# NVlabs/CenterPose

Measured on NVIDIA H100. Metric: images/sec at 512x512 DLA-34 (dla_34 + DCNv2, 7 heads, decode + PnP), higher is better.
Workload: dtype tf32x3

## Files before the change

### centerpose_b200/csrc/common.cuh

```cuda
#pragma once
#include <cuda_runtime.h>
#include <stdint.h>
#include <stdio.h>
#include <string>

#include "../../include/centerpose_b200.h"

namespace cp {

void set_error(const std::string& msg);
int fail(int code, const std::string& msg);
extern thread_local long long g_launch_counter;

#define CP_CUDA_CHECK(expr)                                                              \
  do {                                                                                   \
    cudaError_t _e = (expr);                                                             \
    if (_e != cudaSuccess)                                                               \
      return ::cp::fail(CP_ERR_CUDA, std::string(#expr) + ": " + cudaGetErrorString(_e)); \
  } while (0)

#define CP_LAUNCH_CHECK(what)                                                            \
  do {                                                                                   \
    cudaError_t _e = cudaGetLastError();                                                 \
    if (_e != cudaSuccess)                                                               \
// ... 40 lines not shown
  const float* fuse_b[16];
  float* fuse_out[16];
  int fuse_cout[16];
  int ipm;
  long long wstride, tstride;
  unsigned nchw_per_model;
};
inline int model_ipm(const IgemmParams& p) { return p.ipm > 0 ? p.ipm : p.B; }

int launch_igemm_fp32(const IgemmParams& p, cudaStream_t stream);

int decode_pnp_models(const cp_decode_params* prm, int models, const cp_heads* heads, const double* meta, float* dets,
                      float* poses, int32_t* n_valid, void* workspace, size_t workspace_bytes, void* stream);

struct LaunchInfo {
  int BN = 0;
  int ksplit = 1;
  long long grid = 0;
};

bool conv3_c16_supported(const IgemmParams& p);
int launch_conv3_c16(const IgemmParams& p, cudaStream_t stream);
bool stem_supported(const IgemmParams& p);
int launch_stem_conv(const IgemmParams& p, cudaStream_t s);

struct ConvKernel {
  int family = CP_FAM_IGEMM_FP32;
  bool x3 = false;
  bool round_out = false;
  int BN = 0;
  int cslab = 0;
  size_t wbytes = 0;
};
struct ConvPolicy {
  bool small_on_cuda_cores;
  bool dcn_tma;
  bool round_out;
  bool cuda_core_fallback;
};
inline bool known_precision(int32_t precision) {
  return precision == CP_PREC_FP32 || precision == CP_PREC_TF32X3 || precision == CP_PREC_BF16 || precision == CP_PREC_TF32;
}
inline bool gather_x3(int32_t precision) { return precision == CP_PREC_TF32 || precision == CP_PREC_TF32X3; }
ConvKernel select_conv_kernel(const IgemmParams& p, int32_t precision, const ConvPolicy& pol);
struct alignas(64) TmaMaps {
  unsigned char map[4][128];
};
int conv_encode(const ConvKernel& k, const IgemmParams& p, int Bmax, TmaMaps* maps);
int conv_pack(const ConvKernel& k, const IgemmParams& p, int ld, void* tiles, cudaStream_t s);
int conv_launch(const ConvKernel& k, const IgemmParams& p, const TmaMaps* maps, cudaStream_t s, LaunchInfo* info = nullptr);
int run_conv(IgemmParams& p, int32_t precision, const ConvPolicy& pol, cudaStream_t s);

int splitk_factor(long long tiles, int slabs, int num_sms, size_t tile_floats, size_t ws_floats);

bool umma_supported(const IgemmParams& p, int prec);
int umma_tile_n(int CoutPad, int prec);
size_t umma_weight_bytes(int Kreal, int CoutPad, int prec);
int launch_pack_umma_weight(const float* src_k_by_ld, int ld, int Kreal, int Cout, int CoutPad, int prec, void* dst,
                            cudaStream_t s);
int launch_igemm_umma(const IgemmParams& p, int prec, cudaStream_t stream, LaunchInfo* info = nullptr);

int launch_maxpool2(const float* in, float* out, int B, int H, int W, int C, cudaStream_t s);
int launch_maxpool3s2(const float* in, const float* residual, float* out, int B, int H, int W, int C, cudaStream_t s);
int launch_pack_deconv_weight(const float* w_io44, const float* scale, float* out, int Cin, int Cout, int CoutPad, int Kpad,
                              cudaStream_t s);
int launch_upsample_add(const float* in, const float* wgt_kkc, const float* skip, float* out, int B,
                        int Hin, int Win, int C, int f, cudaStream_t s, int ipm = 0, long long wstride = 0);
int launch_pack_conv_weight(const float* w_oihw, const float* scale, float* out, int Cout, int Cin,
                            int kh, int kw, int CoutPad, int Kpad, int ld, int colOff, cudaStream_t s,
                            int CinPad = 0);
int launch_pack_bias(const float* conv_bias, const float* bn_w, const float* bn_b, const float* bn_mean,
                     const float* bn_var, float* scale_out, float* bias_out, int C, int CPad, float eps,
                     cudaStream_t s);
int launch_pack_up_weight(const float* w_c1kk, float* out_kkc, int C, int k, cudaStream_t s);
int launch_nchw_to_nhwc(const float* in, float* out, int B, int C, int H, int W, int outStride,
                        int chanOffset, cudaStream_t s);
int launch_nhwc_to_nchw(const float* in, float* out, int B, int C, int H, int W, int inStride, cudaStream_t s);
constexpr int kGnBlocks = 64, kGnMaxGroups = 64;
inline size_t gn_workspace_doubles(int B) { return (size_t)B * kGnMaxGroups * 2 * (1 + kGnBlocks); }
int launch_group_norm_relu(float* x, const float* gamma, const float* beta, int B, int HW, int C,
                           int stride, int chanOffset, int groups, float eps, double* ws, cudaStream_t s, int ipm = 0,
                           long long wstride = 0);
int launch_gru_gates(const float* xi, const float* hh, const float* hprev, float* hout, int B_HW, int C,
                     int first_step, cudaStream_t s);

constexpr int kX3GroupBlocks = 1;

bool tma_conv_supported(const IgemmParams& p, int x3);
size_t tma_weight_bytes(int Cin, int taps, int CoutPad, int x3);
int tma_tile_n(int CoutPad, int x3);
int tma_cslab(const IgemmParams& p, int x3);
int launch_pack_tma_weight(const float* src_k_by_ld, int ld, int Cin, int taps, int Cout, int CoutPad, int x3, int cslab,
                           int bn, void* dst, cudaStream_t s);
int tma_encode_nhwc_box(const float* base, int C, int W, int H, int B, int strideFloats, int boxC, int boxW, int boxH,
                        int swizzle64, void* map_out );
int tma_conv_encode(const IgemmParams& p, int Bmax, int cslab, void* maps_out );
int launch_conv_tma(const IgemmParams& p, const void* maps, const ConvKernel& k, cudaStream_t stream, LaunchInfo* info);

bool dcn_tma_supported(const IgemmParams& p, int x3);
int dcn_tma_tile_n(int CoutPad, int x3);
int dcn_tma_encode(const IgemmParams& p, int Bmax, void* map_out );
int launch_dcn_tma(const IgemmParams& p, const void* map, const ConvKernel& k, cudaStream_t stream, LaunchInfo* info);

inline int round_up(int x, int m) { return (x + m - 1) / m * m; }

extern thread_local int g_pdl;
// ... 45 lines not shown
```

### centerpose_b200/csrc/conv_select.cu

```cuda
#include <stdlib.h>

#include "common.cuh"

namespace cp {

ConvKernel select_conv_kernel(const IgemmParams& p, int32_t precision, const ConvPolicy& pol) {
  const bool small = p.mode == IGEMM_NCHW_SCALAR || p.Cin < 32;
  if (precision != CP_PREC_FP32 && !(pol.small_on_cuda_cores && small)) {
    const bool tma = precision == CP_PREC_TF32 || precision == CP_PREC_TF32X3;
    const bool x3 = precision == CP_PREC_TF32X3;
    if (tma && pol.dcn_tma && dcn_tma_supported(p, x3))
      return {CP_FAM_DCN_TMA, x3, pol.round_out && !x3, dcn_tma_tile_n(p.CoutPad, x3), 16,
              tma_weight_bytes(p.Cin, 9, p.CoutPad, x3)};
    if (tma && tma_conv_supported(p, x3))
      return {CP_FAM_CONV_TMA, x3, pol.round_out && !x3, tma_tile_n(p.CoutPad, x3), tma_cslab(p, x3),
              tma_weight_bytes(p.Cin, p.kh * p.kw, p.CoutPad, x3)};
    const bool gx3 = gather_x3(precision);
    const int phases = p.mode == IGEMM_DECONV ? 4 : 1;
    if (umma_supported(p, gx3))
      return {CP_FAM_IGEMM_UMMA, gx3, false, umma_tile_n(p.CoutPad, gx3), 0,
              phases * umma_weight_bytes(p.kh * p.kw * p.Cin, p.CoutPad, gx3)};
    if (!pol.cuda_core_fallback) return {CP_FAM_NONE};
  }
  return {stem_supported(p) ? CP_FAM_STEM : (conv3_c16_supported(p) ? CP_FAM_CONV3_C16 : CP_FAM_IGEMM_FP32)};
// ... 12 lines not shown
      return launch_pack_tma_weight(p.wgt, ld, p.Cin, p.kh * p.kw, p.Cout, p.CoutPad, k.x3, k.cslab, k.BN, tiles, s);
    case CP_FAM_IGEMM_UMMA: {
      const int phases = p.mode == IGEMM_DECONV ? 4 : 1;
      const size_t phase_bytes = k.wbytes / phases;
      for (int ph = 0; ph < phases; ++ph)
        if (int rc = launch_pack_umma_weight(p.wgt + (size_t)ph * p.Kpad * ld, ld, p.kh * p.kw * p.Cin, p.Cout, p.CoutPad,
                                             k.x3, (unsigned char*)tiles + ph * phase_bytes, s))
          return rc;
      return CP_OK;
    }
    default:
      return CP_OK;
  }
}

int conv_launch(const ConvKernel& k, const IgemmParams& p, const TmaMaps* maps, cudaStream_t s, LaunchInfo* info) {
  switch (k.family) {
    case CP_FAM_DCN_TMA: return launch_dcn_tma(p, maps->map, k, s, info);
    case CP_FAM_CONV_TMA: return launch_conv_tma(p, maps->map, k, s, info);
    case CP_FAM_IGEMM_UMMA: return launch_igemm_umma(p, k.x3, s, info);
    case CP_FAM_STEM: return launch_stem_conv(p, s);
    case CP_FAM_CONV3_C16: return launch_conv3_c16(p, s);
    case CP_FAM_IGEMM_FP32: return launch_igemm_fp32(p, s);
    default: return fail(CP_ERR_INVALID, "conv: no kernel selected");
  }
}

int run_conv(IgemmParams& p, int32_t precision, const ConvPolicy& pol, cudaStream_t s) {
  const ConvKernel k = select_conv_kernel(p, precision, pol);
  if (k.family == CP_FAM_NONE) return fail(CP_ERR_INVALID, "shape not supported by the wgmma kernel");
  if (!k.wbytes) return conv_launch(k, p, nullptr, s);
  void* tiles = nullptr;
  CP_CUDA_CHECK(cudaMallocAsync(&tiles, k.wbytes, s));
  TmaMaps maps;
  int rc = conv_encode(k, p, p.B, &maps);
  if (!rc) rc = conv_pack(k, p, p.CoutPad, tiles, s);
  if (!rc) {
    p.wgt_umma = tiles;
    rc = conv_launch(k, p, &maps, s);
  }
  cudaFreeAsync(tiles, s);
  return rc;
}

int splitk_factor(long long tiles, int slabs, int num_sms, size_t tile_floats, size_t ws_floats) {
  const char* off = getenv("CP_NO_SPLITK");
  if (!ws_floats || (off && atoi(off) != 0)) return 1;
  int S = 1;
  for (int cand = 2; cand <= slabs; ++cand)
    if (slabs % cand == 0 && tiles * cand <= num_sms && (size_t)tiles * cand * tile_floats <= ws_floats) S = cand;
  return S;
}

}
```

### centerpose_b200/csrc/conv_tma.cu

```cuda
#include <cuda.h>

#include "common.cuh"
#include "umma_common.cuh"

namespace cp {
namespace {

constexpr int TM_BM = 128;
constexpr int TM_THREADS = 384;
constexpr int TM_THREADS_X3 = 512;

struct TmaConvParams {
  CUtensorMap amap[4];
  int nsrc;
  int srcC[4];
  int B, H, W, Cin, Cout, CoutPad, BN;
  int k;
  int tile_m;
  int Wt, boxh;
  int tiles_per_image;
  long long total_tiles;
  long long m_tiles;
  uint32_t slab_bytes, slab_stride;
  int SA, SB;
  const float* bias;
  const float* residual;
  int resStride, relu, res_after_relu;
  float* out;
  int outStride, out_nchw;
  int round_tf32;
  int cslab;
  int x3;
  int group;
  const unsigned char* wtiles;
  int ksplit, sps;
  float* part;
  int fuse, tph;
  const float* fuse_w[16];
  const float* fuse_b[16];
  float* fuse_out[16];
  int fuse_cout[16];
  int ipm;
  long long wstride, tstride, tiles_per_model;
};

using namespace umma;

struct TmaCtl {
  unsigned long long a_full[4], a_empty[4], a_split[4];
  unsigned long long b_full[8], b_empty[8];
};
static_assert(sizeof(TmaCtl) <= 512, "control block");

struct TileGeo {
  int n_tile, img, g0, r_lo, model;
  long long pos0;
};
template <bool MULTI>
__device__ __forceinline__ TileGeo decode_tile(const TmaConvParams& p, long long ct, int n_tiles) {
  TileGeo g;
  g.n_tile = (int)(ct % n_tiles);
  const long long m_tile = ct / n_tiles;
  g.img = 0;
  g.g0 = 0;
  g.r_lo = 0;
  g.pos0 = 0;
  g.model = 0;
  if (p.k == 3) {
    g.img = (int)(m_tile / p.tiles_per_image);
    g.g0 = (int)(m_tile - (long long)g.img * p.tiles_per_image) * p.tile_m;
    const int t = g.g0 - 1;
    g.r_lo = (t >= 0) ? t / p.Wt : -((-t + p.Wt - 1) / p.Wt);
    if (MULTI) g.model = g.img / p.ipm;
  } else if (MULTI) {
    g.model = (int)(m_tile / p.tiles_per_model);
    g.pos0 = (long long)g.model * p.ipm * p.H * p.W + (m_tile - g.model * p.tiles_per_model) * p.tile_m;
  } else {
    g.pos0 = m_tile * p.tile_m;
  }
  return g;
}

template <bool MULTI>
__device__ __forceinline__ bool tile_position(const TmaConvParams& p, const TileGeo& g, int i, int* n, int* oy, int* ox, int* m) {
  bool valid;
  if (p.k == 3) {
// ... 137 lines not shown
              h.y = tf32_round(v[u].y); l.y = tf32_round(v[u].y - h.y);
              h.z = tf32_round(v[u].z); l.z = tf32_round(v[u].z - h.z);
              h.w = tf32_round(v[u].w); l.w = tf32_round(v[u].w - h.w);
              st_shared_v4f(hi + ((c0 + u * 128) << 4), h.x, h.y, h.z, h.w);
              st_shared_v4f(lo + ((c0 + u * 128) << 4), l.x, l.y, l.z, l.w);
            }
          }
        }
        fence_proxy_async_smem();
        mbar_arrive(smem_u32(&ctl->a_split[stage]));
        if (++stage == p.SA) {
          stage = 0;
          phase ^= 1u;
        }
      }
    }
  } else {
    if (X3) asm volatile("setmaxnreg.inc.sync.aligned.u32 208;");
    const int c = (warp - 4) >> 2, wt = tid & 127;
    float* dstage = reinterpret_cast<float*>(smem + (drain0 - smem_u32(smem))) + (size_t)c * (DRAIN_STAGE_BYTES / 4);
    const uint32_t bar_a = smem_u32(X3 ? &ctl->a_split[0] : &ctl->a_full[0]);
    const uint32_t bar_a_empty = smem_u32(&ctl->a_empty[0]);
    const uint32_t bar_b_full = smem_u32(&ctl->b_full[0]), bar_b_empty = smem_u32(&ctl->b_empty[0]);
    const uint32_t a_lo_u = p.slab_stride >> 4, b_lo_u = ((uint32_t)BN * rowb) >> 4;
    EpiParams ep;
    ep.bias = p.bias;
    ep.residual = p.residual;
    ep.resStride = p.resStride;
    ep.relu = p.relu;
    ep.res_after_relu = p.res_after_relu;
    ep.round_tf32 = p.round_tf32;
    ep.out = p.out;
    ep.outStride = p.outStride;
    ep.out_nchw = p.out_nchw;
    ep.Cout = p.Cout;
    ep.CoutPad = p.CoutPad;
    ep.H = p.H;
    ep.W = p.W;
    int sa = 0, sb = 0;
    uint32_t pa = 0, pb = 0;
    float acc[BN / 2];
    float sums[X3 ? BN / 2 : 1];
    float acc2[FUSE ? 16 : 1];
#pragma unroll
    for (int j = 0; j < BN / 2; ++j) acc[j] = 0.f;
#pragma unroll
    for (int j = 0; j < (FUSE ? 16 : 1); ++j) acc2[j] = 0.f;
    for (long long it = 0, tile = tile_at(0); tile < total_tiles; tile = tile_at(++it)) {
      const TileGeo g = decode_tile<MULTI>(p, tile / KS_SPLIT, n_tiles);
      const uint32_t row0 = (p.k == 3 ? (uint32_t)(g.g0 - 1 - g.r_lo * p.Wt) : 0u) + (uint32_t)c * 64u;
#pragma unroll
      for (int j = 0; j < (X3 ? BN / 2 : 1); ++j) sums[j] = 0.f;
      int kbi = 0, gk = 0;
      for (int s = 0; s < sps; ++s) {
        mbar_wait(bar_a + 8u * (uint32_t)sa, pa);
        const uint32_t a_slab = slabs0 + (uint32_t)sa * a_stage;
        for (int tap = 0; tap < taps; ++tap, ++kbi) {
          const int ky = tap / 3, kx = tap - ky * 3;
          const uint32_t arow = row0 + (p.k == 3 ? (uint32_t)(ky * p.Wt + kx) : 0u);
          mbar_wait(bar_b_full + 8u * (uint32_t)sb, pb);
          const uint64_t da = make_desc(a_slab + arow * rowb, p.cslab);
          const uint64_t db = make_desc(btiles0 + (uint32_t)sb * btile_bytes, p.cslab);
          const bool fresh = X3 ? gk == 0 : kbi == 0;
          if (p.cslab == 32)
            mma_kblock<BN, X3, false, 4>(acc, da, db, a_lo_u, b_lo_u, fresh);
          else
            mma_kblock<BN, X3, false, 2>(acc, da, db, a_lo_u, b_lo_u, fresh);
          if (wt == 0) {
            mbar_arrive(bar_b_empty + 8u * (uint32_t)sb);
            if (tap == taps - 1) mbar_arrive(bar_a_empty + 8u * (uint32_t)sa);
          }
          if (++sb == p.SB) {
            sb = 0;
            pb ^= 1u;
          }
          if (X3) {
            if (gk == p.group - 1 || kbi == KB - 1) {
#pragma unroll
              for (int j = 0; j < (X3 ? BN / 2 : 1); ++j) sums[j] += acc[X3 ? j : 0];
              gk = 0;
            } else {
              ++gk;
            }
          }
        }
        if (++sa == p.SA) {
          sa = 0;
          pa ^= 1u;
        }
      }
      const int r_me = wt >> 1;
      int n, oy, ox, m;
      const bool valid = tile_position<MULTI>(p, g, c * 64 + r_me, &n, &oy, &ox, &m);
      const int col_end = min(p.Cout, (g.n_tile + 1) * BN);
      const int head = FUSE ? g.n_tile / p.tph : 0, part = FUSE ? g.n_tile - head * p.tph : 0;
      const size_t wofs = MULTI ? (size_t)g.model * p.wstride : 0;
      if (MULTI) ep.bias = p.bias + wofs;
      if (FUSE && part == 0) {
#pragma unroll
        for (int j = 0; j < (FUSE ? 16 : 1); ++j) acc2[j] = 0.f;
      }
      auto fn = [&](int r, int cb, float (&v)[16]) {
        if (cb >= BN) return;
        if (!FUSE && KS_SPLIT > 1) {
          const long long mn = tile / KS_SPLIT;
          const int ks = (int)(tile % KS_SPLIT);
          float4* mine = reinterpret_cast<float4*>(p.part) + (((size_t)mn * KS_SPLIT + ks) * (BN >> 2) + (cb >> 2)) * p.tile_m +
                         c * 64 + r;
#pragma unroll
          for (int q = 0; q < 4; ++q) __stcg(mine + (size_t)q * p.tile_m, make_float4(v[4 * q], v[4 * q + 1], v[4 * q + 2], v[4 * q + 3]));
        } else if (FUSE) {
          const float* b1 = p.bias + wofs + (size_t)g.n_tile * BN + cb;
          const float4* w2 = reinterpret_cast<const float4*>(p.fuse_w[head] + wofs) + ((size_t)part * BN + cb) * 4;
#pragma unroll
          for (int q = 0; q < 16; ++q) {
            const float h = fmaxf(v[q] + __ldg(b1 + q), 0.f);
#pragma unroll
            for (int u = 0; u < 4; ++u) {
              const float4 w = __ldg(w2 + q * 4 + u);
              acc2[FUSE ? 4 * u + 0 : 0] = fmaf(h, w.x, acc2[FUSE ? 4 * u + 0 : 0]);
              acc2[FUSE ? 4 * u + 1 : 0] = fmaf(h, w.y, acc2[FUSE ? 4 * u + 1 : 0]);
              acc2[FUSE ? 4 * u + 2 : 0] = fmaf(h, w.z, acc2[FUSE ? 4 * u + 2 : 0]);
              acc2[FUSE ? 4 * u + 3 : 0] = fmaf(h, w.w, acc2[FUSE ? 4 * u + 3 : 0]);
            }
          }
        } else {
          epilogue_row<16>(ep, v, valid, m, n, oy, ox, g.n_tile * BN + cb, col_end);
        }
      };
      if constexpr (X3)
        drain_rows<BN>(sums, dstage, wt, 1 + c, fn);
      else
        drain_rows<BN>(acc, dstage, wt, 1 + c, fn);
      if (FUSE && part == p.tph - 1) {
#pragma unroll
        for (int j = 0; j < (FUSE ? 16 : 1); ++j) acc2[j] += __shfl_xor_sync(0xffffffffu, acc2[j], 1);
        if ((wt & 1) == 0 && valid) {
          const int co = p.fuse_cout[head];
          float* o = p.fuse_out[head] + ((size_t)n * co * p.H + oy) * p.W + ox;
          const size_t plane = (size_t)p.H * p.W;
#pragma unroll
          for (int j = 0; j < 16; ++j)
            if (j < co) o[j * plane] = acc2[FUSE ? j : 0] + __ldg(p.fuse_b[head] + wofs + j);
// ... 203 lines not shown
  cudaLaunchConfig_t cfg = cfg0;
  cudaLaunchAttribute attr[1];
  attr[0].id = cudaLaunchAttributeProgrammaticStreamSerialization;
  attr[0].val.programmaticStreamSerializationAllowed = 1;
  cfg.attrs = attr;
  cfg.numAttrs = g_pdl ? 1 : 0;
  CP_CUDA_CHECK(cudaLaunchKernelEx(&cfg, kern, q));
  CP_LAUNCH_CHECK("conv_tma_kernel");
  return CP_OK;
}

int launch_conv_tma(const IgemmParams& p, const void* maps, const ConvKernel& k, cudaStream_t stream, LaunchInfo* info) {
  if (!p.wgt_umma) return fail(CP_ERR_INVALID, "conv_tma: weight tiles missing");
  if (p.B % model_ipm(p)) return fail(CP_ERR_INVALID, "conv_tma: batch is not a whole number of models");
  const bool x3 = k.x3;
  TmaConvParams q;
  memset(&q, 0, sizeof(q));
  memcpy(q.amap, maps, sizeof(CUtensorMap) * 4);
  q.nsrc = p.nsrc;
  for (int s = 0; s < 4; ++s) q.srcC[s] = p.srcC[s];
  q.B = p.B;
  q.H = p.Hin;
  q.W = p.Win;
  q.Cin = p.Cin;
  q.Cout = p.Cout;
  q.CoutPad = p.CoutPad;
  q.BN = k.BN;
  q.x3 = x3;
  q.cslab = k.cslab;
  q.group = kX3GroupBlocks * (32 / q.cslab);
  q.k = p.kh;
  q.Wt = p.Win + 2;
  q.tile_m = TM_BM;
  q.boxh = tma_boxh(q.Wt);
  q.ipm = model_ipm(p);
  q.wstride = p.wstride;
  q.tstride = p.tstride;
  size_t m_tiles;
  if (q.k == 3) {
    q.tiles_per_image = (p.Hin * q.Wt + q.tile_m - 1) / q.tile_m;
    m_tiles = (size_t)q.tiles_per_image * p.B;
    q.slab_bytes = (uint32_t)q.boxh * q.Wt * (uint32_t)q.cslab * 4u;
  } else {
    q.tiles_per_image = 0;
    q.tiles_per_model = ((long long)q.ipm * p.Hin * p.Win + q.tile_m - 1) / q.tile_m;
    m_tiles = (size_t)q.tiles_per_model * (p.B / q.ipm);
    q.slab_bytes = (uint32_t)q.tile_m * (uint32_t)q.cslab * 4u;
  }
  q.slab_stride = (q.slab_bytes + 1023u) & ~1023u;
  const uint32_t btile = (uint32_t)q.BN * (uint32_t)q.cslab * 4u * (x3 ? 2u : 1u);
  const uint32_t a_stage = q.slab_stride * (x3 ? 2u : 1u);
  size_t smem = 0;
  if (int rc = tma_smem_layout(a_stage, btile, q.k, &q.SA, &q.SB, &smem)) return rc;
  q.bias = p.bias;
  q.residual = p.residual;
  q.resStride = p.resStride;
  q.relu = p.relu;
  q.res_after_relu = p.res_after_relu;
  q.out = p.out;
  q.outStride = p.outStride;
  q.out_nchw = p.out_nchw;
  q.round_tf32 = k.round_out;
  q.wtiles = (const unsigned char*)p.wgt_umma;
  if (p.fuse_n > 0) {
    if (p.fuse_hidden % q.BN || p.CoutPad != p.fuse_n * p.fuse_hidden || !p.relu || p.residual || (x3 && q.BN != 128))
      return fail(CP_ERR_INVALID, "conv_tma: fused 1x1 needs relu, no residual and head_conv a multiple of the N tile");
    q.fuse = 1;
    q.tph = p.fuse_hidden / q.BN;
    for (int h = 0; h < p.fuse_n; ++h) {
      q.fuse_w[h] = p.fuse_w[h];
      q.fuse_b[h] = p.fuse_b[h];
      q.fuse_out[h] = p.fuse_out[h];
      q.fuse_cout[h] = p.fuse_cout[h];
    }
  }
  q.m_tiles = (long long)m_tiles;
  q.part = p.splitk_ws;
  const long long mn = (long long)m_tiles * (p.CoutPad / q.BN);
  const int nslab = q.Cin / q.cslab;
  int num_sms = 0;
  if (int rc = device_sm_count(&num_sms)) return rc;
  q.ksplit = x3 && !q.fuse ? splitk_factor(mn, nslab, num_sms, (size_t)q.tile_m * q.BN, p.splitk_ws_floats) : 1;
  q.sps = nslab / q.ksplit;
  q.total_tiles = mn * q.ksplit;
  if (q.total_tiles >= (1ll << 31)) return fail(CP_ERR_INVALID, "conv_tma: too many tiles");
  cudaLaunchConfig_t cfg{};
  cfg.gridDim = dim3((unsigned)(q.total_tiles < num_sms ? q.total_tiles : num_sms));
  cfg.blockDim = dim3(x3 ? TM_THREADS_X3 : TM_THREADS);
  cfg.dynamicSmemBytes = smem;
  cfg.stream = stream;
  const bool multi = p.B > q.ipm;
  int rc;
  if (multi)
    rc = x3 ? (q.fuse ? launch_conv_tma_kernel<true, true, true>(q, cfg) : launch_conv_tma_kernel<true, false, true>(q, cfg))
            : (q.fuse ? launch_conv_tma_kernel<false, true, true>(q, cfg) : launch_conv_tma_kernel<false, false, true>(q, cfg));
  else
    rc = x3 ? (q.fuse ? launch_conv_tma_kernel<true, true, false>(q, cfg) : launch_conv_tma_kernel<true, false, false>(q, cfg))
            : (q.fuse ? launch_conv_tma_kernel<false, true, false>(q, cfg) : launch_conv_tma_kernel<false, false, false>(q, cfg));
  if (rc) return rc;
  if (info) {
    info->BN = q.BN;
    info->ksplit = q.ksplit;
    info->grid = cfg.gridDim.x;
  }
  if (q.ksplit > 1) {
    const long long threads = mn * (q.BN / 4) * q.tile_m;
// ... 9 lines not shown
```

### centerpose_b200/csrc/umma_common.cuh

```cuda
#pragma once
#include <cuda.h>
#include <cuda_runtime.h>
#include <stdint.h>
#include <stdio.h>

namespace cp {
namespace umma {

__device__ __forceinline__ uint32_t smem_u32(const void* p) { return (uint32_t)__cvta_generic_to_shared(p); }

__device__ __forceinline__ void mbar_init(uint32_t bar, uint32_t count) {
  asm volatile("mbarrier.init.shared::cta.b64 [%0], %1;" ::"r"(bar), "r"(count));
}
__device__ __forceinline__ void mbar_arrive(uint32_t bar) {
  asm volatile("mbarrier.arrive.shared::cta.b64 _, [%0];" ::"r"(bar) : "memory");
}
__device__ __forceinline__ void mbar_arrive_expect_tx(uint32_t bar, uint32_t bytes) {
  asm volatile("mbarrier.arrive.expect_tx.shared::cta.b64 _, [%0], %1;" ::"r"(bar), "r"(bytes) : "memory");
}
__device__ __forceinline__ bool mbar_try_wait(uint32_t bar, uint32_t parity) {
  uint32_t ok;
  asm volatile(
      "{\n\t.reg .pred p;\n\tmbarrier.try_wait.parity.shared::cta.b64 p, [%1], %2;\n\tselp.b32 %0, 1, 0, p;\n\t}"
      : "=r"(ok)
// ... 83 lines not shown
template <> __device__ __forceinline__ void wgmma_bf16<64>(float (&d)[32], uint64_t da, uint64_t db, uint32_t scale_d) {
  asm volatile(
      "{\n\t.reg .pred p;\n\tsetp.ne.b32 p, %34, 0;\n\t"
      "wgmma.mma_async.sync.aligned.m64n64k16.f32.bf16.bf16 {%0,%1,%2,%3,%4,%5,%6,%7,%8,%9,%10,%11,%12,%13,%14,%15,%16,%17,%18,%19,%20,%21,%22,%23,%24,%25,%26,%27,%28,%29,%30,%31}, %32, %33, p, 1, 1, 0, 0;\n\t}"
      : "+f"(d[0]), "+f"(d[1]), "+f"(d[2]), "+f"(d[3]), "+f"(d[4]), "+f"(d[5]), "+f"(d[6]), "+f"(d[7]), "+f"(d[8]), "+f"(d[9]), "+f"(d[10]), "+f"(d[11]), "+f"(d[12]), "+f"(d[13]), "+f"(d[14]), "+f"(d[15]), "+f"(d[16]), "+f"(d[17]), "+f"(d[18]), "+f"(d[19]), "+f"(d[20]), "+f"(d[21]), "+f"(d[22]), "+f"(d[23]), "+f"(d[24]), "+f"(d[25]), "+f"(d[26]), "+f"(d[27]), "+f"(d[28]), "+f"(d[29]), "+f"(d[30]), "+f"(d[31])
      : "l"(da), "l"(db), "r"(scale_d));
}
template <> __device__ __forceinline__ void wgmma_bf16<128>(float (&d)[64], uint64_t da, uint64_t db, uint32_t scale_d) {
  asm volatile(
      "{\n\t.reg .pred p;\n\tsetp.ne.b32 p, %66, 0;\n\t"
      "wgmma.mma_async.sync.aligned.m64n128k16.f32.bf16.bf16 {%0,%1,%2,%3,%4,%5,%6,%7,%8,%9,%10,%11,%12,%13,%14,%15,%16,%17,%18,%19,%20,%21,%22,%23,%24,%25,%26,%27,%28,%29,%30,%31,%32,%33,%34,%35,%36,%37,%38,%39,%40,%41,%42,%43,%44,%45,%46,%47,%48,%49,%50,%51,%52,%53,%54,%55,%56,%57,%58,%59,%60,%61,%62,%63}, %64, %65, p, 1, 1, 0, 0;\n\t}"
      : "+f"(d[0]), "+f"(d[1]), "+f"(d[2]), "+f"(d[3]), "+f"(d[4]), "+f"(d[5]), "+f"(d[6]), "+f"(d[7]), "+f"(d[8]), "+f"(d[9]), "+f"(d[10]), "+f"(d[11]), "+f"(d[12]), "+f"(d[13]), "+f"(d[14]), "+f"(d[15]), "+f"(d[16]), "+f"(d[17]), "+f"(d[18]), "+f"(d[19]), "+f"(d[20]), "+f"(d[21]), "+f"(d[22]), "+f"(d[23]), "+f"(d[24]), "+f"(d[25]), "+f"(d[26]), "+f"(d[27]), "+f"(d[28]), "+f"(d[29]), "+f"(d[30]), "+f"(d[31]), "+f"(d[32]), "+f"(d[33]), "+f"(d[34]), "+f"(d[35]), "+f"(d[36]), "+f"(d[37]), "+f"(d[38]), "+f"(d[39]), "+f"(d[40]), "+f"(d[41]), "+f"(d[42]), "+f"(d[43]), "+f"(d[44]), "+f"(d[45]), "+f"(d[46]), "+f"(d[47]), "+f"(d[48]), "+f"(d[49]), "+f"(d[50]), "+f"(d[51]), "+f"(d[52]), "+f"(d[53]), "+f"(d[54]), "+f"(d[55]), "+f"(d[56]), "+f"(d[57]), "+f"(d[58]), "+f"(d[59]), "+f"(d[60]), "+f"(d[61]), "+f"(d[62]), "+f"(d[63])
      : "l"(da), "l"(db), "r"(scale_d));
}
template <> __device__ __forceinline__ void wgmma_bf16<256>(float (&d)[128], uint64_t da, uint64_t db, uint32_t scale_d) {
  asm volatile(
      "{\n\t.reg .pred p;\n\tsetp.ne.b32 p, %130, 0;\n\t"
      "wgmma.mma_async.sync.aligned.m64n256k16.f32.bf16.bf16 {%0,%1,%2,%3,%4,%5,%6,%7,%8,%9,%10,%11,%12,%13,%14,%15,%16,%17,%18,%19,%20,%21,%22,%23,%24,%25,%26,%27,%28,%29,%30,%31,%32,%33,%34,%35,%36,%37,%38,%39,%40,%41,%42,%43,%44,%45,%46,%47,%48,%49,%50,%51,%52,%53,%54,%55,%56,%57,%58,%59,%60,%61,%62,%63,%64,%65,%66,%67,%68,%69,%70,%71,%72,%73,%74,%75,%76,%77,%78,%79,%80,%81,%82,%83,%84,%85,%86,%87,%88,%89,%90,%91,%92,%93,%94,%95,%96,%97,%98,%99,%100,%101,%102,%103,%104,%105,%106,%107,%108,%109,%110,%111,%112,%113,%114,%115,%116,%117,%118,%119,%120,%121,%122,%123,%124,%125,%126,%127}, %128, %129, p, 1, 1, 0, 0;\n\t}"
      : "+f"(d[0]), "+f"(d[1]), "+f"(d[2]), "+f"(d[3]), "+f"(d[4]), "+f"(d[5]), "+f"(d[6]), "+f"(d[7]), "+f"(d[8]), "+f"(d[9]), "+f"(d[10]), "+f"(d[11]), "+f"(d[12]), "+f"(d[13]), "+f"(d[14]), "+f"(d[15]), "+f"(d[16]), "+f"(d[17]), "+f"(d[18]), "+f"(d[19]), "+f"(d[20]), "+f"(d[21]), "+f"(d[22]), "+f"(d[23]), "+f"(d[24]), "+f"(d[25]), "+f"(d[26]), "+f"(d[27]), "+f"(d[28]), "+f"(d[29]), "+f"(d[30]), "+f"(d[31]), "+f"(d[32]), "+f"(d[33]), "+f"(d[34]), "+f"(d[35]), "+f"(d[36]), "+f"(d[37]), "+f"(d[38]), "+f"(d[39]), "+f"(d[40]), "+f"(d[41]), "+f"(d[42]), "+f"(d[43]), "+f"(d[44]), "+f"(d[45]), "+f"(d[46]), "+f"(d[47]), "+f"(d[48]), "+f"(d[49]), "+f"(d[50]), "+f"(d[51]), "+f"(d[52]), "+f"(d[53]), "+f"(d[54]), "+f"(d[55]), "+f"(d[56]), "+f"(d[57]), "+f"(d[58]), "+f"(d[59]), "+f"(d[60]), "+f"(d[61]), "+f"(d[62]), "+f"(d[63]), "+f"(d[64]), "+f"(d[65]), "+f"(d[66]), "+f"(d[67]), "+f"(d[68]), "+f"(d[69]), "+f"(d[70]), "+f"(d[71]), "+f"(d[72]), "+f"(d[73]), "+f"(d[74]), "+f"(d[75]), "+f"(d[76]), "+f"(d[77]), "+f"(d[78]), "+f"(d[79]), "+f"(d[80]), "+f"(d[81]), "+f"(d[82]), "+f"(d[83]), "+f"(d[84]), "+f"(d[85]), "+f"(d[86]), "+f"(d[87]), "+f"(d[88]), "+f"(d[89]), "+f"(d[90]), "+f"(d[91]), "+f"(d[92]), "+f"(d[93]), "+f"(d[94]), "+f"(d[95]), "+f"(d[96]), "+f"(d[97]), "+f"(d[98]), "+f"(d[99]), "+f"(d[100]), "+f"(d[101]), "+f"(d[102]), "+f"(d[103]), "+f"(d[104]), "+f"(d[105]), "+f"(d[106]), "+f"(d[107]), "+f"(d[108]), "+f"(d[109]), "+f"(d[110]), "+f"(d[111]), "+f"(d[112]), "+f"(d[113]), "+f"(d[114]), "+f"(d[115]), "+f"(d[116]), "+f"(d[117]), "+f"(d[118]), "+f"(d[119]), "+f"(d[120]), "+f"(d[121]), "+f"(d[122]), "+f"(d[123]), "+f"(d[124]), "+f"(d[125]), "+f"(d[126]), "+f"(d[127])
      : "l"(da), "l"(db), "r"(scale_d));
}

template <int N>
__device__ __forceinline__ void wgmma_tf32_rs(float (&d)[N / 2], const uint32_t (&a)[4], uint64_t db, uint32_t scale_d);
template <> __device__ __forceinline__ void wgmma_tf32_rs<16>(float (&d)[8], const uint32_t (&a)[4], uint64_t db, uint32_t scale_d) {
  asm volatile(
      "{\n\t.reg .pred p;\n\tsetp.ne.b32 p, %13, 0;\n\t"
      "wgmma.mma_async.sync.aligned.m64n16k8.f32.tf32.tf32 {%0,%1,%2,%3,%4,%5,%6,%7}, {%8,%9,%10,%11}, %12, p, 1, 1;\n\t}"
      : "+f"(d[0]), "+f"(d[1]), "+f"(d[2]), "+f"(d[3]), "+f"(d[4]), "+f"(d[5]), "+f"(d[6]), "+f"(d[7])
      : "r"(a[0]), "r"(a[1]), "r"(a[2]), "r"(a[3]), "l"(db), "r"(scale_d));
}
template <> __device__ __forceinline__ void wgmma_tf32_rs<32>(float (&d)[16], const uint32_t (&a)[4], uint64_t db, uint32_t scale_d) {
  asm volatile(
      "{\n\t.reg .pred p;\n\tsetp.ne.b32 p, %21, 0;\n\t"
      "wgmma.mma_async.sync.aligned.m64n32k8.f32.tf32.tf32 {%0,%1,%2,%3,%4,%5,%6,%7,%8,%9,%10,%11,%12,%13,%14,%15}, {%16,%17,%18,%19}, %20, p, 1, 1;\n\t}"
      : "+f"(d[0]), "+f"(d[1]), "+f"(d[2]), "+f"(d[3]), "+f"(d[4]), "+f"(d[5]), "+f"(d[6]), "+f"(d[7]), "+f"(d[8]), "+f"(d[9]), "+f"(d[10]), "+f"(d[11]), "+f"(d[12]), "+f"(d[13]), "+f"(d[14]), "+f"(d[15])
      : "r"(a[0]), "r"(a[1]), "r"(a[2]), "r"(a[3]), "l"(db), "r"(scale_d));
}
template <> __device__ __forceinline__ void wgmma_tf32_rs<64>(float (&d)[32], const uint32_t (&a)[4], uint64_t db, uint32_t scale_d) {
  asm volatile(
      "{\n\t.reg .pred p;\n\tsetp.ne.b32 p, %37, 0;\n\t"
      "wgmma.mma_async.sync.aligned.m64n64k8.f32.tf32.tf32 {%0,%1,%2,%3,%4,%5,%6,%7,%8,%9,%10,%11,%12,%13,%14,%15,%16,%17,%18,%19,%20,%21,%22,%23,%24,%25,%26,%27,%28,%29,%30,%31}, {%32,%33,%34,%35}, %36, p, 1, 1;\n\t}"
      : "+f"(d[0]), "+f"(d[1]), "+f"(d[2]), "+f"(d[3]), "+f"(d[4]), "+f"(d[5]), "+f"(d[6]), "+f"(d[7]), "+f"(d[8]), "+f"(d[9]), "+f"(d[10]), "+f"(d[11]), "+f"(d[12]), "+f"(d[13]), "+f"(d[14]), "+f"(d[15]), "+f"(d[16]), "+f"(d[17]), "+f"(d[18]), "+f"(d[19]), "+f"(d[20]), "+f"(d[21]), "+f"(d[22]), "+f"(d[23]), "+f"(d[24]), "+f"(d[25]), "+f"(d[26]), "+f"(d[27]), "+f"(d[28]), "+f"(d[29]), "+f"(d[30]), "+f"(d[31])
      : "r"(a[0]), "r"(a[1]), "r"(a[2]), "r"(a[3]), "l"(db), "r"(scale_d));
}
template <> __device__ __forceinline__ void wgmma_tf32_rs<128>(float (&d)[64], const uint32_t (&a)[4], uint64_t db, uint32_t scale_d) {
  asm volatile(
      "{\n\t.reg .pred p;\n\tsetp.ne.b32 p, %69, 0;\n\t"
      "wgmma.mma_async.sync.aligned.m64n128k8.f32.tf32.tf32 {%0,%1,%2,%3,%4,%5,%6,%7,%8,%9,%10,%11,%12,%13,%14,%15,%16,%17,%18,%19,%20,%21,%22,%23,%24,%25,%26,%27,%28,%29,%30,%31,%32,%33,%34,%35,%36,%37,%38,%39,%40,%41,%42,%43,%44,%45,%46,%47,%48,%49,%50,%51,%52,%53,%54,%55,%56,%57,%58,%59,%60,%61,%62,%63}, {%64,%65,%66,%67}, %68, p, 1, 1;\n\t}"
      : "+f"(d[0]), "+f"(d[1]), "+f"(d[2]), "+f"(d[3]), "+f"(d[4]), "+f"(d[5]), "+f"(d[6]), "+f"(d[7]), "+f"(d[8]), "+f"(d[9]), "+f"(d[10]), "+f"(d[11]), "+f"(d[12]), "+f"(d[13]), "+f"(d[14]), "+f"(d[15]), "+f"(d[16]), "+f"(d[17]), "+f"(d[18]), "+f"(d[19]), "+f"(d[20]), "+f"(d[21]), "+f"(d[22]), "+f"(d[23]), "+f"(d[24]), "+f"(d[25]), "+f"(d[26]), "+f"(d[27]), "+f"(d[28]), "+f"(d[29]), "+f"(d[30]), "+f"(d[31]), "+f"(d[32]), "+f"(d[33]), "+f"(d[34]), "+f"(d[35]), "+f"(d[36]), "+f"(d[37]), "+f"(d[38]), "+f"(d[39]), "+f"(d[40]), "+f"(d[41]), "+f"(d[42]), "+f"(d[43]), "+f"(d[44]), "+f"(d[45]), "+f"(d[46]), "+f"(d[47]), "+f"(d[48]), "+f"(d[49]), "+f"(d[50]), "+f"(d[51]), "+f"(d[52]), "+f"(d[53]), "+f"(d[54]), "+f"(d[55]), "+f"(d[56]), "+f"(d[57]), "+f"(d[58]), "+f"(d[59]), "+f"(d[60]), "+f"(d[61]), "+f"(d[62]), "+f"(d[63])
      : "r"(a[0]), "r"(a[1]), "r"(a[2]), "r"(a[3]), "l"(db), "r"(scale_d));
}

template <int BN, bool X3, bool BF16, int KS>
__device__ __forceinline__ void mma_kblock(float (&acc)[BN / 2], uint64_t da, uint64_t db, uint32_t a_lo, uint32_t b_lo,
                                           bool fresh) {
  wg_fence();
#pragma unroll
  for (int ks = 0; ks < KS; ++ks) {
    const uint32_t sd = (fresh && ks == 0) ? 0u : 1u;
    if (X3) {
      wgmma_tf32<BN>(acc, da + a_lo + 2u * ks, db + 2u * ks, sd);
      wgmma_tf32<BN>(acc, da + 2u * ks, db + b_lo + 2u * ks, 1u);
    } else if (BF16) {
      wgmma_bf16<BN>(acc, da + 2u * ks, db + 2u * ks, sd);
    } else {
      wgmma_tf32<BN>(acc, da + 2u * ks, db + 2u * ks, sd);
    }
  }
  if (X3) {
#pragma unroll
    for (int ks = 0; ks < KS; ++ks) wgmma_tf32<BN>(acc, da + 2u * ks, db + 2u * ks, 1u);
  }
  wg_commit();
  wg_wait<0>();
}

__device__ __forceinline__ float tf32_round(float x) {
  return __uint_as_float((__float_as_uint(x) + 0x1000u) & 0xffffe000u);
}
__device__ __forceinline__ void ldsm_x4(uint32_t (&r)[4], uint32_t addr) {
  asm volatile("ldmatrix.sync.aligned.m8n8.x4.shared.b16 {%0, %1, %2, %3}, [%4];"
               : "=r"(r[0]), "=r"(r[1]), "=r"(r[2]), "=r"(r[3])
               : "r"(addr));
}

template <int BN, int KS>
__device__ __forceinline__ void mma_kblock_x3(float (&acc)[BN / 2], uint32_t a_tile, int wt, uint64_t db, uint32_t b_lo,
                                              bool fresh) {
  const uint32_t lane = (uint32_t)wt & 31u;
  const uint32_t row = (uint32_t)(wt >> 5) * 16u + (lane & 7u) + ((lane >> 3) & 1u) * 8u;
  const uint32_t a_row = a_tile + row * (32u * KS);
  const uint32_t x = ((lane >> 4) << 4) ^ ((a_row >> 3) & (KS == 4 ? 0x70u : 0x30u));
  uint32_t hi[KS][4], lo[KS][4];
#pragma unroll
  for (int ks = 0; ks < KS; ++ks) {
    ldsm_x4(hi[ks], a_row + (((uint32_t)ks << 5) ^ x));
#pragma unroll
    for (int j = 0; j < 4; ++j) {
      const float v = __uint_as_float(hi[ks][j]);
      const float h = tf32_round(v);
      lo[ks][j] = __float_as_uint(tf32_round(v - h));
      hi[ks][j] = __float_as_uint(h);
    }
  }
  wg_fence();
#pragma unroll
  for (int ks = 0; ks < KS; ++ks) {
    wgmma_tf32_rs<BN>(acc, lo[ks], db + 2u * ks, (fresh && ks == 0) ? 0u : 1u);
    wgmma_tf32_rs<BN>(acc, hi[ks], db + b_lo + 2u * ks, 1u);
  }
#pragma unroll
  for (int ks = 0; ks < KS; ++ks) wgmma_tf32_rs<BN>(acc, hi[ks], db + 2u * ks, 1u);
  wg_commit();
  wg_wait<0>();
#pragma unroll
  for (int ks = 0; ks < KS; ++ks)
#pragma unroll
    for (int j = 0; j < 4; ++j) asm volatile("" : "+r"(hi[ks][j]), "+r"(lo[ks][j]));
}

__device__ __forceinline__ uint32_t pack_bf16x2(float a, float b) {
  uint32_t r;
  asm("cvt.rn.bf16x2.f32 %0, %1, %2;" : "=r"(r) : "f"(b), "f"(a));
  return r;
}
__device__ __forceinline__ void st_shared_v4(uint32_t addr, uint32_t a, uint32_t b, uint32_t c, uint32_t d) {
// ... 152 lines not shown
```

Before: 583.2.

## Overlap consecutive wgmma K-blocks in TMA conv by deferring wait and slot release

The TMA conv kernel now issues each K-block's wgmma group and waits only for the previous group (wait<1>) before releasing that group's shared-memory ring slots. Before, it waited for every group to finish. This keeps the tensor cores fed across K-block boundaries instead of draining the pipeline after each block. The overlap is on by default and can be turned off with the CP_KBLOCK_SYNC env var. It needs ring depth of at least 2, and the slot release and tf32x3 group-sum logic become more intricate, which raises the risk of ordering mistakes.

After: 587.0, median of 6. No clear change (+0.7%).

```diff
diff --git a/centerpose_b200/csrc/common.cuh b/centerpose_b200/csrc/common.cuh
--- a/centerpose_b200/csrc/common.cuh
+++ b/centerpose_b200/csrc/common.cuh
@@ -116,6 +116,7 @@
 int run_conv(IgemmParams& p, int32_t precision, const ConvPolicy& pol, cudaStream_t s);
 
 int splitk_factor(long long tiles, int slabs, int num_sms, size_t tile_floats, size_t ws_floats);
+bool kblock_sync();
 
 bool umma_supported(const IgemmParams& p, int prec);
 int umma_tile_n(int CoutPad, int prec);
diff --git a/centerpose_b200/csrc/conv_select.cu b/centerpose_b200/csrc/conv_select.cu
--- a/centerpose_b200/csrc/conv_select.cu
+++ b/centerpose_b200/csrc/conv_select.cu
@@ -88,4 +88,9 @@
   return S;
 }
 
+bool kblock_sync() {
+  const char* e = getenv("CP_KBLOCK_SYNC");
+  return e && atoi(e) != 0;
 }
+
+}
diff --git a/centerpose_b200/csrc/conv_tma.cu b/centerpose_b200/csrc/conv_tma.cu
--- a/centerpose_b200/csrc/conv_tma.cu
+++ b/centerpose_b200/csrc/conv_tma.cu
@@ -32,6 +32,7 @@
   int cslab;
   int x3;
   int group;
+  int overlap;
   const unsigned char* wtiles;
   int ksplit, sps;
   float* part;
@@ -275,6 +276,7 @@
 #pragma unroll
       for (int j = 0; j < (X3 ? BN / 2 : 1); ++j) sums[j] = 0.f;
       int kbi = 0, gk = 0;
+      bool held = false;
       for (int s = 0; s < sps; ++s) {
         mbar_wait(bar_a + 8u * (uint32_t)sa, pa);
         const uint32_t a_slab = slabs0 + (uint32_t)sa * a_stage;
@@ -286,19 +288,32 @@
           const uint64_t db = make_desc(btiles0 + (uint32_t)sb * btile_bytes, p.cslab);
           const bool fresh = X3 ? gk == 0 : kbi == 0;
           if (p.cslab == 32)
-            mma_kblock<BN, X3, false, 4>(acc, da, db, a_lo_u, b_lo_u, fresh);
+            mma_kblock_issue<BN, X3, false, 4>(acc, da, db, a_lo_u, b_lo_u, fresh);
           else
-            mma_kblock<BN, X3, false, 2>(acc, da, db, a_lo_u, b_lo_u, fresh);
-          if (wt == 0) {
-            mbar_arrive(bar_b_empty + 8u * (uint32_t)sb);
-            if (tap == taps - 1) mbar_arrive(bar_a_empty + 8u * (uint32_t)sa);
+            mma_kblock_issue<BN, X3, false, 2>(acc, da, db, a_lo_u, b_lo_u, fresh);
+          if (held) {
+            wg_wait_acc<1>(acc);
+            if (wt == 0) {
+              mbar_arrive(bar_b_empty + 8u * (uint32_t)(sb == 0 ? p.SB - 1 : sb - 1));
+              if (tap == 0) mbar_arrive(bar_a_empty + 8u * (uint32_t)(sa == 0 ? p.SA - 1 : sa - 1));
+            }
+          }
+          const bool group_end = X3 ? (gk == p.group - 1 || kbi == KB - 1) : kbi == KB - 1;
+          held = !group_end && p.overlap > (tap == taps - 1 ? 1 : 0);
+          if (!held) {
+            wg_wait_acc<0>(acc);
+            if (wt == 0) {
+              mbar_arrive(bar_b_empty + 8u * (uint32_t)sb);
+              if (tap == taps - 1) mbar_arrive(bar_a_empty + 8u * (uint32_t)sa);
+            }
           }
           if (++sb == p.SB) {
             sb = 0;
             pb ^= 1u;
           }
           if (X3) {
-            if (gk == p.group - 1 || kbi == KB - 1) {
+            if (group_end) {
+              wg_wait_acc<0>(acc);
 #pragma unroll
               for (int j = 0; j < (X3 ? BN / 2 : 1); ++j) sums[j] += acc[X3 ? j : 0];
               gk = 0;
@@ -312,6 +327,8 @@
           pa ^= 1u;
         }
       }
+      wg_wait<0>();
+      if (!X3) wg_wait_acc<0>(acc);
       const int r_me = wt >> 1;
       int n, oy, ox, m;
       const bool valid = tile_position<MULTI>(p, g, c * 64 + r_me, &n, &oy, &ox, &m);
@@ -621,6 +638,9 @@
   const uint32_t a_stage = q.slab_stride * (x3 ? 2u : 1u);
   size_t smem = 0;
   if (int rc = tma_smem_layout(a_stage, btile, q.k, &q.SA, &q.SB, &smem)) return rc;
+  q.overlap = kblock_sync() ? 0 : (q.SA >= 2 ? 2 : 1);
+  if (q.overlap && (q.SB < 2 || (q.overlap == 2 && q.SA < 2)))
+    return fail(CP_ERR_INVALID, "conv_tma: K-block overlap over a one-stage ring");
   q.bias = p.bias;
   q.residual = p.residual;
   q.resStride = p.resStride;
diff --git a/centerpose_b200/csrc/umma_common.cuh b/centerpose_b200/csrc/umma_common.cuh
--- a/centerpose_b200/csrc/umma_common.cuh
+++ b/centerpose_b200/csrc/umma_common.cuh
@@ -159,9 +159,16 @@
       : "r"(a[0]), "r"(a[1]), "r"(a[2]), "r"(a[3]), "l"(db), "r"(scale_d));
 }
 
+template <int N, int R>
+__device__ __forceinline__ void wg_wait_acc(float (&acc)[R]) {
+  wg_wait<N>();
+#pragma unroll
+  for (int j = 0; j < R; ++j) asm volatile("" : "+f"(acc[j]));
+}
+
 template <int BN, bool X3, bool BF16, int KS>
-__device__ __forceinline__ void mma_kblock(float (&acc)[BN / 2], uint64_t da, uint64_t db, uint32_t a_lo, uint32_t b_lo,
-                                           bool fresh) {
+__device__ __forceinline__ void mma_kblock_issue(float (&acc)[BN / 2], uint64_t da, uint64_t db, uint32_t a_lo,
+                                                 uint32_t b_lo, bool fresh) {
   wg_fence();
 #pragma unroll
   for (int ks = 0; ks < KS; ++ks) {
@@ -180,6 +187,11 @@
     for (int ks = 0; ks < KS; ++ks) wgmma_tf32<BN>(acc, da + 2u * ks, db + 2u * ks, 1u);
   }
   wg_commit();
+}
+template <int BN, bool X3, bool BF16, int KS>
+__device__ __forceinline__ void mma_kblock(float (&acc)[BN / 2], uint64_t da, uint64_t db, uint32_t a_lo, uint32_t b_lo,
+                                           bool fresh) {
+  mma_kblock_issue<BN, X3, BF16, KS>(acc, da, db, a_lo, b_lo, fresh);
   wg_wait<0>();
 }
 
```
